# mqcomplab/bblean

Hardware: AMD Instinct MI355X
Metric: fingerprints/sec clustered (2048-bit, thr=0.3) (higher is better)
Workload: dtype u8

## Files before the change

bblean_amd/_engine.py:

```python
from __future__ import annotations

import ctypes as C
import os
import typing as tp

import numpy as np
from numpy.typing import NDArray

from bblean_amd import _lib

_WIDTH_DTYPES = {1: np.uint8, 2: np.uint16, 4: np.uint32, 8: np.uint64}


def _is_device_tensor(x: object) -> bool:
    return hasattr(x, "data_ptr") and getattr(x, "is_cuda", False)


def _launch_stream(x: object) -> int | None:
    if not _is_device_tensor(x):
        return None
    import torch

    return int(torch.cuda.current_stream(x.device).cuda_stream)

# ... 310 lines not shown
        out = np.empty((pos.size, self.nbytes), dtype=np.uint8)
        if pos.size:
            _lib.check(self._lib.bbh_tree_gather_centroids(self._h, pos.ctypes.data, pos.size, out.ctypes.data))
        return out

    def stats(self) -> NDArray[np.uint64]:
        out = np.zeros(8, dtype=np.uint64)
        _lib.check(self._lib.bbh_tree_stats(self._h, out.ctypes.data))
        return out

    def kernel_counts(self) -> NDArray[np.uint64]:
        out = np.zeros(8, dtype=np.uint64)
        _lib.check(self._lib.bbh_tree_kernel_counts(self._h, out.ctypes.data))
        return out

    def sys_counts(self) -> NDArray[np.uint64]:
        out = np.zeros(8, dtype=np.uint64)
        _lib.check(self._lib.bbh_tree_sys_counts(self._h, out.ctypes.data))
        return out

    def memory(self) -> NDArray[np.uint64]:
        out = np.zeros(8, dtype=np.uint64)
        _lib.check(self._lib.bbh_tree_memory(self._h, out.ctypes.data))
        return out

    def compact(self, seal: bool = True) -> None:
        _lib.check(self._lib.bbh_tree_compact(self._h, 1 if seal else 0))

    @staticmethod
    def image_min_stage(n_features: int) -> int:
# ... 49 lines not shown
```

bblean_amd/_lib.py:

```python
from __future__ import annotations

import ctypes as C
import os
from pathlib import Path

import numpy as np

_LIB: C.CDLL | None = None
_HERE = Path(__file__).resolve().parent

BBH_OK = 0
BBH_ERR_INVALID = 1
BBH_ERR_HIP = 2
BBH_ERR_NO_DEVICE = 3
BBH_ERR_CAPACITY = 4
BBH_ERR_STATE = 5
BBH_TOPK_MAX = 64

_vp = C.c_void_p
_i32 = C.c_int32
_i64 = C.c_int64
_f64 = C.c_double
_int = C.c_int

# ... 26 lines not shown
    ),
    "bbh_tree_create": (_int, [C.POINTER(_vp), _i32, _f64, _i32, _f64, _vp, _i64, _i32, _i32]),
    "bbh_tree_destroy": (_int, [_vp]),
    "bbh_tree_set_merge": (_int, [_vp, _i32, _f64, _vp, _i64, _f64, _i32]),
    "bbh_tree_reset": (_int, [_vp]),
    "bbh_tree_fit_packed": (_int, [_vp, _vp, _i64, _i64, _vp, _vp]),
    "bbh_tree_fit_buffers": (_int, [_vp, _vp, _i32, _i64, _vp, _vp]),
    "bbh_trees_fit_packed": (_int, [_vp, _i32, _vp, _vp, _vp, _vp, _vp]),
    "bbh_trees_fit_buffers": (_int, [_vp, _i32, _vp, _vp, _vp, _vp, _vp]),
    "bbh_tree_leaf_count": (_int, [_vp, C.POINTER(_i64)]),
    "bbh_tree_export_leaves": (_int, [_vp, _vp, _vp, _vp, _vp, _i32]),
    "bbh_tree_gather_buffers": (_int, [_vp, _vp, _i64, _i32, _vp]),
    "bbh_tree_gather_centroids": (_int, [_vp, _vp, _i64, _vp]),
    "bbh_tree_stats": (_int, [_vp, _vp]),
    "bbh_tree_kernel_counts": (_int, [_vp, _vp]),
    "bbh_tree_sys_counts": (_int, [_vp, _vp]),
    "bbh_tree_memory": (_int, [_vp, _vp]),
    "bbh_tree_compact": (_int, [_vp, _i32]),
    "bbh_tree_save_fd": (_int, [_vp, _int, C.c_uint64, C.POINTER(C.c_uint64)]),
    "bbh_tree_load_fd": (_int, [C.POINTER(_vp), _int, _i32, C.c_uint64]),
    "bbh_tree_image_check_fd": (_int, [_int, C.POINTER(C.c_uint64)]),
    "bbh_profile_enable": (_int, [_int]),
    "bbh_profile_reset": (_int, []),
    "bbh_profile_get": (_int, [C.c_char_p, C.POINTER(_i64), C.POINTER(_f64)]),
    "bbh_profile_units": (_int, [C.c_char_p, C.POINTER(_i64)]),
    "bbh_profile_longest": (_int, [C.c_char_p, C.POINTER(_f64), C.POINTER(_i64)]),
}

EXPORTED_SYMBOLS = tuple(_PROTOTYPES)

# ... 79 lines not shown
```

bblean_amd/csrc/bb_tree.hip:

```cpp
#include "bb_common.h"

#include <atomic>
#include <chrono>

#include <rocprim/device/device_scan.hpp>

#include <algorithm>
#include <cmath>
#include <future>
#include <type_traits>

using namespace bbd;

namespace {

constexpr int TB = 256;
constexpr int TW = TB / 64;
constexpr uint32_t NONE = 0xFFFFFFFFu;
constexpr int MAXD = 256;
constexpr int MAXFAST = 5;
constexpr int NRED = 2 + MAXFAST;
constexpr int MAX_BF = 1023;
constexpr int NPLW = 9;
constexpr int SPLIT_MLP = 16;
// ... 43 lines not shown
    uint32_t* node_link;
    RowMeta* node_rm;
    NodeHdr* node_hdr;
    uint8_t* scratch_cent;
    uint8_t* cf8;
    uint16_t* cf16;
    uint32_t* cf32;
    uint32_t cap_nodes, cap8, cap16, cap32;
    uint32_t ctr[C_COUNT];
    unsigned long long stats[8];
    unsigned long long phase[16];
    unsigned long long sphase[8];
    unsigned long long splitprof[10];
    unsigned long long mlprof[8];
    unsigned long long rprof[4];
    const uint8_t* rows;
    long long row_stride;
    const uint8_t* bufs;
    int32_t width;
    int32_t use_root_cache;
    long long n_elems;
    uint32_t* out_leaf;
    long long processed;
    int32_t stop_reason;
    int32_t audit;
    uint32_t giveup_line;
};

struct Smem {
    uint32_t x, vec, cA, cB;
// ... 2320 lines not shown
    if (!t->lazy_pools) {
        BB_HIP(hipMemset(h.node_hdr, 0, ((size_t)h.cap_nodes + 1) * sizeof(NodeHdr)));
        BB_TRY(write_empty_root(h));
    }
    h.ctr[C_NODES] = nblk;
    h.ctr[C_N8] = 1;
    h.ctr[C_ROOT] = 0;
    h.ctr[C_FIRST_LEAF] = 0;
    h.ctr[C_DEPTH] = 1;
    std::memset(h.stats, 0, sizeof(h.stats));
    std::memset(h.phase, 0, sizeof(h.phase));
    std::memset(h.sphase, 0, sizeof(h.sphase));
    std::memset(h.splitprof, 0, sizeof(h.splitprof));
    std::memset(h.mlprof, 0, sizeof(h.mlprof));
    std::memset(h.rprof, 0, sizeof(h.rprof));
    h.stats[5] = 1;
    t->chain_valid = false;
    t->pipe_ml = false;
    t->unsup_stretch = 0;
    return BBH_OK;
}

int set_tol(bbh_tree* t, const double* tab, int64_t len) {
    double* fresh = nullptr;
    if (tab && len > 0) {
        BB_HIP(bb::dev_alloc(&fresh, (size_t)len * 8));
        const hipError_t e = hipMemcpy(fresh, tab, (size_t)len * 8, hipMemcpyHostToDevice);
        if (e != hipSuccess) {
            (void)bb::dev_free(fresh);
            BB_HIP(e);
// ... 143 lines not shown
static void print_pipe_phases(const bbh_tree* t) {
    static const char* nm[16] = {"router:setup", "router:wait", "router:compare", "router:commit", "router:drain", "leaf:wait", "leaf:fill",
                                 "leaf:compare", "leaf:cf+dot", "leaf:decide+apply", "all:flush", "all:cold", "#runs", "#router-stale", "#leaf-pre-hits", "#leaf-stale"};
    const double n = (double)(t->h.stats[2] + t->h.stats[3]);
    fprintf(stderr, "[bbhip pipe phases, per insert]");
    for (int i = 0; i < 16; ++i) fprintf(stderr, " %s=%.*f", nm[i], i < 12 ? 0 : 4, n > 0 ? (double)t->h.phase[i] / n : 0.0);
    static const char* kd[3] = {"pre-compared, best row folded", "own", "pre-compared, every row checked"};
    fprintf(stderr, "\n[bbhip pipe leaf compares]");
    for (int i = 0; i < 3; ++i)
        fprintf(stderr, " %s: %.3f/insert x %.0f cycles", kd[i], n > 0 ? (double)t->h.sphase[2 * i + 1] / n : 0.0,
                t->h.sphase[2 * i + 1] ? (double)t->h.sphase[2 * i] / (double)t->h.sphase[2 * i + 1] : 0.0);
    fprintf(stderr, "\n");
    fprintf(stderr, "[bbhip pipe router waits, per insert] ring entry %.0f, row + pre-compare of wave 2 %.0f, pending jobs of a nearly full leaf %.0f, "
            "decision on a full leaf %.0f\n", n > 0 ? (double)t->h.rprof[0] / n : 0.0, n > 0 ? (double)t->h.rprof[1] / n : 0.0,
            n > 0 ? (double)t->h.rprof[2] / n : 0.0, n > 0 ? (double)t->h.rprof[3] / n : 0.0);
    if (t->h.splitprof[8]) {
        const double ns = (double)t->h.splitprof[8];
        fprintf(stderr, "[bbhip pipe leaf splits] %.4f/insert x %.0f cycles:", n > 0 ? ns / n : 0.0, (double)t->h.splitprof[9] / ns);
        for (int i = 0; i < 8; ++i) fprintf(stderr, " s%d=%.0f", i, (double)t->h.splitprof[i] / ns);
        fprintf(stderr, "\n");
    }
    if (t->pipe_ml)
        fprintf(stderr, "[bbhip pipe multi-level router] upper-slot fills %.3f/insert x %.0f cycles; tracking levels committed %.3f/insert, "
                "cluster-feature cache misses %.3f/insert; router waiting for a level's update by a helper wave %.0f cycles/insert, for "
                "all of them and their stores (before a fill) %.0f; of a fill: loads %.0f cycles, slot + corrections %.0f\n", n > 0 ? (double)t->h.sphase[7] / n : 0.0,
                t->h.sphase[7] ? (double)t->h.sphase[6] / (double)t->h.sphase[7] : 0.0, n > 0 ? (double)t->h.mlprof[1] / n : 0.0,
                n > 0 ? (double)t->h.mlprof[0] / n : 0.0, n > 0 ? (double)t->h.mlprof[2] / n : 0.0, n > 0 ? (double)t->h.mlprof[3] / n : 0.0,
                t->h.sphase[7] ? (double)t->h.mlprof[4] / (double)t->h.sphase[7] : 0.0, t->h.sphase[7] ? (double)t->h.mlprof[5] / (double)t->h.sphase[7] : 0.0);
}

// ... 232 lines not shown
            else if (left_midway == 0) multi_chunk = std::min<long long>(2 * multi_chunk, 1ll << 18);
        }

        for (size_t a = 0; a < active.size() && rc == BBH_OK; ++a) {
            Job& j = jobs[active[a]];
            bbh_tree* t = j.t;
            TreeDev& h = t->h;
            const TreeDev& back = harr[a];
            std::memcpy(h.ctr, back.ctr, sizeof(h.ctr));
            std::memcpy(h.stats, back.stats, sizeof(h.stats));
            std::memcpy(h.phase, back.phase, sizeof(h.phase));
            std::memcpy(h.sphase, back.sphase, sizeof(h.sphase));
            std::memcpy(h.splitprof, back.splitprof, sizeof(h.splitprof));
            std::memcpy(h.mlprof, back.mlprof, sizeof(h.mlprof));
            std::memcpy(h.rprof, back.rprof, sizeof(h.rprof));
            j.done += back.processed;
            t->kcount[label.kcol] += (uint64_t)back.processed;
            t->kcount[3 + label.kcol] += 1;
            if (engine == Engine::Sys) {
                rc = sys_after_launch(t, back, s);
                if (rc != BBH_OK) break;
            }
            const bool pool_stop = back.stop_reason == STOP_NODES || back.stop_reason == STOP_CF8 || back.stop_reason == STOP_CF16 || back.stop_reason == STOP_CF32;
            if (back.stop_reason == STOP_PIPE_UNSUPPORTED) t->kcount[6] += 1;
            if (pool_stop) t->kcount[7] += 1;
            if (j.old_left > 0) j.old_left = std::max<int64_t>(0, j.old_left - back.processed);
            if (t->sys_off_left > 0 && engine != Engine::Sys) t->sys_off_left = std::max<int64_t>(0, t->sys_off_left - back.processed);
            if (prof_tok != (size_t)-1) bb::prof_units(prof_tok, back.processed);
            j.stalls = (back.processed == 0 && back.stop_reason != STOP_PIPE_UNSUPPORTED && back.stop_reason != STOP_PIPE_NEEDS_ML) ? j.stalls + 1 : 0;
            if (j.stalls > 3) { rc = bb::fail(BBH_ERR_CAPACITY, "tree engine made no progress (stop reason %d)", back.stop_reason); break; }
// ... 497 lines not shown
}

extern "C" int bbh_tree_gather_centroids(bbh_tree* t, const int64_t* positions, int64_t m, uint8_t* out) {
    if (!t || (m > 0 && (!positions || !out))) return bb::fail(BBH_ERR_INVALID, "null argument");
    if (m < 0) return bb::fail(BBH_ERR_INVALID, "negative position count");
    if (m == 0) return BBH_OK;
    return gather_positions(t, positions, m, 0, nullptr, out);
}

extern "C" int bbh_tree_kernel_counts(bbh_tree* t, uint64_t* out8) {
    if (!t || !out8) return bb::fail(BBH_ERR_INVALID, "null argument");
    for (int i = 0; i < 8; ++i) out8[i] = t->kcount[i];
    return BBH_OK;
}

extern "C" int bbh_tree_sys_counts(bbh_tree* t, uint64_t* out8) {
    if (!t || !out8) return bb::fail(BBH_ERR_INVALID, "null argument");
    for (int i = 0; i < 8; ++i) out8[i] = t->syscount[i];
    return BBH_OK;
}

extern "C" int bbh_tree_memory(bbh_tree* t, uint64_t* out8) {
    if (!t || !out8) return bb::fail(BBH_ERR_INVALID, "null argument");
    const TreeDev& h = t->h;
    const size_t F = (size_t)h.F;
    out8[0] = (uint64_t)h.cap_nodes * block_bytes(h);
    out8[1] = (uint64_t)std::min(h.cap_nodes, h.ctr[C_NODES]) * block_bytes(h);
    out8[2] = (uint64_t)h.cap8 * F + (uint64_t)h.cap16 * F * 2 + (uint64_t)h.cap32 * F * 4;
    out8[3] = std::max(t->peak_bytes, pool_bytes(h));
    out8[4] = t->gc_runs;
// ... 31 lines not shown
```

bblean_amd/csrc/bb_tree_pipe.inc:

```

constexpr int PW_MAX = 8;
__host__ __device__ constexpr int pipe_pw(int bf) { return bf > 63 ? 4 : 8; }
__host__ __device__ constexpr int pipe_prew(int bf) { return bf > 63 ? 2 : 4; }
constexpr int PZ = 6;
constexpr int PNP = 12;
constexpr int PROMO_RESERVE = 1024;
constexpr int STOP_PIPE_UNSUPPORTED = 9;
constexpr int STOP_INTERNAL = 10;
constexpr int STOP_PIPE_NEEDS_ML = 11;
constexpr int STOP_PIPE_PREFERS_SL = 12;
#ifndef BBH_ML_STINT
#define BBH_ML_STINT 256
#endif
constexpr long long PIPE_ML_STINT = BBH_ML_STINT;
constexpr int PEMAX = 4;
constexpr uint32_t PRT = 16;

enum PipeReason : uint32_t { PR_DONE = 0, PR_COLD = 1, PR_STOP = 2, PR_UNSUP = 3, PR_FLUSH = 4, PR_ABORT = 5, PR_SPLIT = 6, PR_NEEDML = 7, PR_PREFSL = 8 };
enum PipeSplit : int { PS_LEAF = 0, PS_P, PS_JP, PS_LENP, PS_TRK, PS_POP, PS_XOFF, PS_SI };
enum PipeCtl : int { PC_HEAD = 0, PC_TAIL, PC_END, PC_ABORT, PC_REASON, PC_E_LO, PC_E_HI, PC_STOPCODE, PC_DCOUNT, PC_NZ, PC_PGO, PC_PLEN, PC_LGO, PC_PZERO,
                     PC_WM,
                     PC_COUNT };
static_assert(PC_COUNT <= 16, "the control block is 16 words");

struct PSmem {
    uint32_t x, ctr, stats;
    uint32_t ctl, ring, res, xq, delta, zrec;
    uint32_t mb, part;
    uint32_t srec;
    uint32_t llog, prec;
    uint32_t pver, lver, preP, preL, pst;
    int pw, prew;
    uint32_t leaf0, lslot_bytes, s_card, s_link, s_rm;
    uint32_t pslot, p_card, p_link, p_n, p_ts, p_clen, p_pend, pslot_bytes;
    uint32_t lrest;
    uint32_t cold_base, total;
    uint32_t cfc;
    uint32_t tcf;
    int nl, ncf, ntc;
    int nus;
    uint32_t upath, urt, urp;
};

__host__ __device__ constexpr PSmem pipe_layout(int bf, int ml = 0) {
    PSmem p{};
    const size_t rows = (size_t)bf + 1;
    p.x = 0; p.ctr = 256; p.stats = 256 + 64;
    uint32_t o = 256 + 64 + 64;
    p.ctl = o; o += 64;
    p.pw = pipe_pw(bf); p.prew = pipe_prew(bf);
    const uint32_t lanes4 = (uint32_t)((rows + 63) / 64 * 256);
    p.ring = o; o += p.pw * 16;
    p.res = o; o += p.pw * 4;
    p.xq = o; o += p.pw * 256;
    p.zrec = o; o += f_align16(PZ * 32);
    p.mb = o; o += 64;
    p.srec = o; o += 32;
    p.pst = o; o += 128;
    p.pver = o; o += lanes4;
    p.preP = o; o += p.prew * lanes4;
    p.part = o; o += 2 * (bf > 63 ? lanes4 : 0u);
    p.leaf0 = f_align16(o);
    p.s_card = f_align16(rows * FRBS);
    p.s_link = p.s_card + f_align16(rows * 4);
    p.s_rm = p.s_link + f_align16(rows * 4);
    p.lslot_bytes = p.s_rm + (uint32_t)(rows * 32);
    p.cold_base = p.leaf0 + p.lslot_bytes;
    p.pslot = p.cold_base;
    p.delta = p.pslot;
    p.p_card = f_align16(rows * FRBS);
    p.p_link = p.p_card + f_align16(rows * 4);
    p.p_n = p.p_link + f_align16(rows * 4);
    p.p_ts = p.p_n + f_align16(rows * 4);
    p.p_clen = p.p_ts + f_align16(rows * 4);
    p.p_pend = p.p_clen + f_align16(rows * 4);
    p.pslot_bytes = p.p_pend + f_align16(rows * 4);
    p.nus = ml ? PEMAX : 1;
    p.lrest = p.pslot + (uint32_t)p.nus * p.pslot_bytes;
    int nl = 1;
    while (nl < (ml ? 3 : 6) && (size_t)p.lrest + (size_t)nl * p.lslot_bytes <= 160 * 1024) ++nl;
    p.nl = nl;
    const uint32_t cold = smem_layout(bf, 256, 0).total;
    const uint32_t end_slots = p.lrest + (uint32_t)(nl - 1) * p.lslot_bytes;
    p.lver = f_align16(end_slots);
    p.preL = bf > 63 ? p.preP : p.lver + (uint32_t)nl * lanes4;
    p.cfc = p.lver + (uint32_t)nl * lanes4 + (bf > 63 ? 0u : (uint32_t)p.prew * lanes4);
    const uint32_t lim = 160 * 1024 - (bf > 63 ? 64u * 7u : 0u) - (ml ? (uint32_t)(PEMAX * 32 + PRT * 8 + PW_MAX * 4 + 64) : 0u);
    int ncf = p.cfc < lim ? (int)((lim - p.cfc) / 2048) : 0;
    p.ncf = ncf > 8 ? 8 : ncf;
    p.tcf = p.cfc + (uint32_t)p.ncf * 2048;
    int ntc = p.tcf < lim ? (int)((lim - p.tcf) / 8192) : 0;
    p.ntc = ntc > 4 ? 4 : (ntc < 0 ? 0 : ntc);
    p.llog = p.tcf + (uint32_t)p.ntc * 8192;
    p.prec = p.llog + 64 * (uint32_t)nl;
    uint32_t end_all = p.prec + 64;
    if (ml) {
        p.upath = end_all;
        p.urt = p.upath + PEMAX * 32;
        p.urp = p.urt + PRT * 8;
        end_all = p.urp + PW_MAX * 4;
    }
    const uint32_t end_cold = p.cold_base + cold;
    p.total = end_all > end_cold ? end_all : end_cold;
    return p;
}

__host__ __device__ constexpr FSmem pipe_fsmem(int bf) {
    const PSmem p = pipe_layout(bf);
    FSmem f{};
    f.x = p.x; f.ctr = p.ctr; f.stats = p.stats;
    f.slot0 = p.leaf0; f.slot_bytes = p.lslot_bytes; f.s_card = p.s_card; f.s_link = p.s_link; f.s_rm = p.s_rm;
    f.cold_base = p.cold_base; f.total = p.total; f.ns = p.nl; f.npp = 0; f.cold_slot = 1;
    return f;
}

static_assert(pipe_layout(50).total <= 160 * 1024, "bf 50 must fit");
static_assert(pipe_layout(254).total <= 160 * 1024, "bf 254 must fit");
static_assert(pipe_layout(50, 1).total <= 160 * 1024 && pipe_layout(50, 1).ntc >= 3 && pipe_layout(50, 1).ncf >= 4 && pipe_layout(50, 1).nl >= 3,
              "bf 50, several exact levels: four upper slots, three leaf slots and the caches must fit");
static_assert(pipe_layout(50, 1).leaf0 == pipe_layout(50).leaf0 && pipe_layout(50, 1).cold_base == pipe_layout(50).cold_base &&
              pipe_layout(50, 1).lslot_bytes == pipe_layout(50).lslot_bytes, "one cold layout per branching factor");

#if defined(__HIPCC__)

#define PIPE_SPIN_LIMIT (1u << 22)
#define PIPE_MARK() ((void)0)
__device__ unsigned int g_pipe_audit = 0;
__device__ unsigned long long g_pipe_audit_runs = 0;
#define PIPE_AUDIT_FAIL(code) atomicCAS(&g_pipe_audit, 0u, ((unsigned)(code) << 16) | (unsigned)__LINE__)
#define PIPE_CBAR() asm volatile("" ::: "memory")

template <int BF>
struct KColdP : KCBase {
    static constexpr bool dynamic_shape = false;
    static constexpr int F = 2048, nb = 256, RB = 256, RBc = 16, RBS = (int)FRBS;
    static constexpr uint32_t rows = BF + 1, bf = BF, nblk = node_blocks(BF + 1);
    static constexpr int nm = 1;
    static constexpr Smem o = smem_layout_cold(BF, pipe_fsmem(BF));
};

template <int BF>
__device__ __attribute__((noinline)) void cold_insert_one_p(unsigned char* smem_raw, TreeDev* T, long long e) {
    tree_insert_body<false, KColdP<BF>, true>(smem_raw, T, e);
}

template <int BF, bool PROF = false>
__device__ __attribute__((noinline)) void cold_leaf_split_p(unsigned char* smem_raw, TreeDev* T, long long e, uint32_t pcx, uint32_t leafnode,
                                                            uint32_t P, uint32_t jp, uint32_t lenP, uint32_t trk) {
    const u64 sp_t0 = PROF ? __builtin_amdgcn_s_memtime() : 0;
    constexpr FSmem f = pipe_fsmem(BF);
    KColdS<BF> k;
    k.cent = T->node_cent; k.card = T->node_card; k.link = T->node_link; k.rm = T->node_rm; k.hdr = T->node_hdr;
    k.scratch = T->scratch_cent; k.cf8 = T->cf8; k.cf16 = T->cf16; k.cf32 = T->cf32;
    k.bufs = nullptr; k.width = 0;
    k.crit = 0; k.tol_len = 0; k.thr = 0; k.tolerance = 0; k.tol = nullptr;
    k.L = (LA unsigned char*)smem_raw;
    k.o = smem_layout_cold(BF, f);
    const int tid = threadIdx.x;
    LA uint32_t* lctr = (LA uint32_t*)(k.L + f.ctr);
    LA uint32_t* bc = lds<uint32_t>(k.L, k.o.bc);
    Elem el;
    el.idx = e; el.nS = 1; el.s1S = 0; el.s2S = 0; el.pcx = pcx;
    __syncthreads();
    uint32_t cN = uni(lctr[C_NODES]), c32 = uni(lctr[C_N32]), cFirst = uni(lctr[C_FIRST_LEAF]);
    int red_slot = 0, cmp_par = 0;
    u64 sph[8] = {0, 0, 0, 0, 0, 0, 0, 0};
    split_node<false, PROF>(k, el, red_slot, cmp_par, leafnode, 0u, true, trk, cN, c32, cFirst, T->ctr, sph);
    const uint32_t node1 = uni(bc[0]), cardA = uni(bc[3]), cardB = uni(bc[4]);
    const uint32_t nA = uni(bc[7]), nB = uni(bc[8]);
    const uint32_t slotA = (2u << 30) | uni(bc[9]), slotB = (2u << 30) | uni(bc[10]);
    const uint32_t bad = uni(bc[11]);
    node_put_row(k, P, jp, k.o.cA, cardA, node1, NONE, nA, slotA, 0, 0);
    node_put_row(k, P, lenP, k.o.cB, cardB, leafnode, NONE, nB, slotB, 0, 0);
    if (tid == 0) {
        stg<uint32_t>(k.hdr + P, lenP + 1);
        lctr[C_NODES] = cN; lctr[C_N32] = c32; lctr[C_FIRST_LEAF] = cFirst;
        lctr[8] = bad ? (uint32_t)STOP_RANGE : (uint32_t)STOP_DONE;
    }
    __syncthreads();
    if constexpr (PROF) {
        if (tid == 0) {
            for (int i = 0; i < 8; ++i) T->splitprof[i] += sph[i];
            T->splitprof[8] += 1;
            T->splitprof[9] += __builtin_amdgcn_s_memtime() - sp_t0;
        }
    }
}

// ... 740 lines not shown
    for (int i = 0; i < 32; ++i) { tx[i] = 0; ty[i] = 0; }
    uint32_t xtag = NONE, xts = 0, ytag = NONE, yts = 0;
    bool curx = false;
    constexpr int NTC = p.ntc;
    uint32_t ttag[NTC > 0 ? NTC : 1], tts[NTC > 0 ? NTC : 1], tuse[NTC > 0 ? NTC : 1];
#pragma unroll
    for (int c = 0; c < (NTC > 0 ? NTC : 1); ++c) { ttag[c] = NONE; tts[c] = 0; tuse[c] = 0; }

    uint32_t Z = 0, zrows = 0, P = NONE, plen = 0;
    constexpr bool RV = RPL == 1;
    uint32_t r_link = NONE, r_n = 0, r_ts = 0, r_clen = 0, r_pend = 0, r_card = 0, r_ver = 0;
    (void)r_link; (void)r_n; (void)r_ts; (void)r_clen; (void)r_pend; (void)r_card; (void)r_ver;
    uint32_t budget = (1u << PNP) - 1;
    bool ok = depth >= 2 && depth - 2 <= (uint32_t)PZ;
    bool needml = false;
    {
        uint32_t nd = cRoot;
#pragma unroll 1
        for (uint32_t z = 0; ok && z + 2 < depth; ++z) {
            const size_t m = (size_t)nd * NG;
            const uint32_t len = uni(ldg<uint32_t>(g_hdr + nd));
            bool any = false;
#pragma unroll
            for (int q = 0; q < RPL; ++q) {
                const uint32_t r = (uint32_t)q * 64 + lane;
                const uint32_t rc = r < rows ? r : rows - 1;
                const uint32_t cd = ldg<uint32_t>(g_card + m + rc);
                any = any || (r < len && cd != 0);
            }
            const u32x4_t r0 = ldg<u32x4_t>((const uint8_t*)(g_rm + m));
            const uint32_t l0 = uni(ldg<uint32_t>(g_link + m));
// ... 9 lines not shown
            const uint32_t zn = uni(zr[0]), zn_at = uni(zr[2]), zfd = uni(zr[3]);
            if (zn == nd && uni(zr[1]) == ts0 && n0 >= zn_at && zfd > (n0 - zn_at) + 64u) {
                fd = zfd - (n0 - zn_at);
            } else {
                uint32_t v[32];
                cf32_lane_load(g_cf32, ts0, lane, v);
                uint32_t mn = 0xFFFFFFFFu;
#pragma unroll
                for (int i = 0; i < 32; ++i) {
                    const uint32_t d = 2u * v[i] < n0 ? n0 - 2u * v[i] : 0u;
                    mn = d < mn ? d : mn;
                }
                fd = wmin32(mn);
                if (lane == 0) { zr[2] = n0; zr[3] = fd; }
            }
            if (lane == 0) { zr[0] = nd; zr[1] = ts0; }
            const uint32_t room = fd > 0 ? fd - 1 : 0;
            budget = room < budget ? room : budget;
            zrows += len;
            nd = l0;
            Z = z + 1;
        }
        P = nd;
    }
    if (!ok) {
        reason = needml ? PR_NEEDML : PR_UNSUP;
    } else if (budget == 0) {
        reason = PR_COLD;
    } else {
        const size_t pm = (size_t)P * NG;
        const u32x2_t hraw = ldg<u32x2_t>(g_hdr + P);
        pipe_fill_rows<K, 0, PFill<K>::NIT>(L, p.pslot, g_cent, P);
        uint32_t lk[RPL];
#pragma unroll
        for (int q = 0; q < RPL; ++q) {
            const uint32_t r = (uint32_t)q * 64 + lane;
            const uint32_t rc = r < rows ? r : rows - 1;
            const uint32_t cd = ldg<uint32_t>(g_card + pm + rc);
            lk[q] = ldg<uint32_t>(g_link + pm + rc);
            const u32x2_t ns = ldg<u32x2_t>((const uint8_t*)(g_rm + pm + rc) + 4);
// ... 29 lines not shown
                const uint32_t rc = r < rows ? r : rows - 1;
                uint32_t cl = bf + 1, clf = 1;
                if (r < plen) {
                    const u32x2_t ch = ldg<u32x2_t>(g_hdr + lk[q]);
                    cl = hw_cap(ch.y) < rows ? bf + 1 : ch.x; clf = ch.y & HW_LEAF;
                }
                bad = bad || clf == 0;
                *(LA uint32_t*)(L + p.pslot + p.p_clen + rc * 4) = cl;
                if constexpr (RV) r_clen = cl;
            }
            if (__ballot(bad) != 0ull) reason = PR_UNSUP;
        }
    }

    pph<PROF>(pr, 0);
    if constexpr (PROF) pr.ph[12] += 1;
    const bool pzero = nzc == 0;
    if (reason == PR_DONE) {
#pragma unroll
        for (int q = 0; q < RPL; ++q) *(LA uint32_t*)(L + p.pver + ((uint32_t)q * 64 + lane) * 4) = 0u;
        if (lane < 8) *(LA uint32_t*)(L + p.pst + lane * 4) = 0u;
        if (lane == 0) {
            *(LA uint32_t*)(L + p.ctl + PC_PLEN * 4) = plen;
            *(LA uint32_t*)(L + p.ctl + PC_PZERO * 4) = pzero ? 1u : 0u;
        }
        PIPE_CBAR();
        lds_st(L, p.ctl + PC_PGO * 4, 1u);
        uint32_t tail_seen = 0;
        auto retire_to_tail = [&]() {
            const uint32_t t = tail_seen;
            PIPE_CBAR();
// ... 258 lines not shown
            if (T->audit != 0 && reason != PR_ABORT) {
                retire_poll();
                asm volatile("s_waitcnt vmcnt(0)" ::: "memory");
                if constexpr (RV) {
                    if (lane < rows) {
                        *(LA uint32_t*)(L + p.pslot + p.p_card + lane * 4) = r_card;
                        *(LA uint32_t*)(L + p.pslot + p.p_n + lane * 4) = r_n;
                        *(LA uint32_t*)(L + p.pslot + p.p_link + lane * 4) = r_link;
                        *(LA uint32_t*)(L + p.pslot + p.p_clen + lane * 4) = r_clen;
                        *(LA uint32_t*)(L + p.pslot + p.p_pend + lane * 4) = r_pend;
                    }
                }
                PIPE_CBAR();
                if (T->audit == 2 && lane == 0) *(LA uint32_t*)(L + p.pslot) ^= 1u;
                pipe_audit_tracking_slot<K>(L, T, p.pslot, P, plen, reason != PR_SPLIT);
            }
        }
        if (xtag != NONE) cf32_lane_store(g_cf32, xts, lane, tx);
        if (ytag != NONE) cf32_lane_store(g_cf32, yts, lane, ty);
#pragma unroll
        for (int c = 0; c < NTC; ++c) {
            if (ttag[c] != NONE) {
                uint32_t* dst = g_cf32 + (size_t)(tts[c] & 0x3FFFFFFFu) * 2048 + (size_t)lane * 32;
#pragma unroll
                for (int g = 0; g < 8; ++g) stg<u32x4_t>(dst + g * 4, *(LA u32x4_t*)(L + p.tcf + (uint32_t)c * 8192 + ((uint32_t)g * 64 + lane) * 16));
            }
        }
#pragma unroll
        for (int k = 0; k < PNP; ++k) *(LA uint32_t*)(L + p.delta + k * 256 + lane * 4) = dp[k];
        pph<PROF>(pr, 4);
// ... 79 lines not shown
        for (uint32_t w = 0; w < 2; ++w) {
            uint32_t spins = 0;
            while (uni(lds_ld(L, p.mb + (CQ_FIN + w) * 4)) != cposted) {
                if (uni(lds_ld(L, p.ctl + PC_ABORT * 4)) != 0u || ++spins > PIPE_SPIN_LIMIT) { lost_c = true; PIPE_MARK(); break; }
            }
        }
        PIPE_CBAR();
        cseen = 0xFFu;
        if constexpr (PROF) cwa_cycles += __builtin_amdgcn_s_memtime() - t0_;
    };
    uint32_t utag = NONE, ulen = 0, uuse = 0, uclock = 0;

    uint32_t Z = 0, zrows = 0, top = NONE;
    uint32_t budget = (1u << PNP) - 1;
    bool ok = depth >= 2;
    {
        uint32_t nd = cRoot;
#pragma unroll 1
        for (uint32_t z = 0; ok && z + 2 < depth && z < (uint32_t)PZ; ++z) {
            const size_t m = (size_t)nd * NG;
            const uint32_t len = uni(ldg<uint32_t>(g_hdr + nd));
            const uint32_t rc = lane < rows ? lane : rows - 1;
            const uint32_t cd = ldg<uint32_t>(g_card + m + rc);
            const bool any = lane < len && cd != 0;
            const u32x4_t r0 = ldg<u32x4_t>((const uint8_t*)(g_rm + m));
            const uint32_t l0 = uni(ldg<uint32_t>(g_link + m));
            if (len == 0) { ok = false; break; }
            if (__ballot(any) != 0ull) break;
            const uint32_t n0 = uni(r0.y), ts0 = uni(r0.z);
            if (n0 >= 0x7FFF0000u) { ok = false; break; }
// ... 2 lines not shown
            const uint32_t zn = uni(zr[0]), zn_at = uni(zr[2]), zfd = uni(zr[3]);
            if (zn == nd && uni(zr[1]) == ts0 && n0 >= zn_at && zfd > (n0 - zn_at) + 64u) {
                fd = zfd - (n0 - zn_at);
            } else {
                uint32_t v[32];
                cf32_lane_load(g_cf32, ts0, lane, v);
                uint32_t mn = 0xFFFFFFFFu;
#pragma unroll
                for (int i = 0; i < 32; ++i) {
                    const uint32_t d = 2u * v[i] < n0 ? n0 - 2u * v[i] : 0u;
                    mn = d < mn ? d : mn;
                }
                fd = wmin32(mn);
                if (lane == 0) { zr[2] = n0; zr[3] = fd; }
            }
            if (lane == 0) { zr[0] = nd; zr[1] = ts0; }
            const uint32_t room = fd > 0 ? fd - 1 : 0;
            budget = room < budget ? room : budget;
            zrows += len;
            nd = l0;
            Z = z + 1;
        }
        top = nd;
    }
    const uint32_t E = ok ? depth - 1 - Z : 0u;

    u64 fprof[2] = {0, 0};
    (void)fprof;
    bool fill_sealed = false;
    auto fill_slot = [&](uint32_t si, uint32_t nd, bool plevel, bool midrun, uint32_t l) -> bool {
        const uint32_t sb = p.pslot + si * p.pslot_bytes;
// ... 894 lines not shown
__device__ __forceinline__ void pipe_flush_delta(LA unsigned char* L, TreeDev* T) {
    constexpr PSmem p = K::p;
    const int tid = threadIdx.x;
    LA uint32_t* ctl = (LA uint32_t*)(L + p.ctl);
    const uint32_t cnt = uni(ctl[PC_DCOUNT]), nz = uni(ctl[PC_NZ]);
    if (cnt == 0 || nz == 0) return;
    uint32_t v[8] = {0, 0, 0, 0, 0, 0, 0, 0};
#pragma unroll
    for (int k = 0; k < PNP; ++k) {
        const uint32_t byte = *(LA uint8_t*)(L + p.delta + k * 256 + tid);
#pragma unroll
        for (int q = 0; q < 8; ++q) v[q] |= ((byte >> (7 - q)) & 1u) << k;
    }
    uint32_t* const g_cf32 = T->cf32;
    RowMeta* const g_rm = T->node_rm;
#pragma unroll 1
    for (uint32_t z = 0; z < nz; ++z) {
        LA uint32_t* zr = (LA uint32_t*)(L + p.zrec + z * 32);
        const uint32_t nd = uni(zr[0]), ts = uni(zr[1]);
        uint32_t* cf = g_cf32 + (size_t)(ts & 0x3FFFFFFFu) * 2048 + (size_t)tid * 8;
        u32x4_t q0 = ldg<u32x4_t>(cf), q1 = ldg<u32x4_t>(cf + 4);
        q0.x += v[0]; q0.y += v[1]; q0.z += v[2]; q0.w += v[3];
        q1.x += v[4]; q1.y += v[5]; q1.z += v[6]; q1.w += v[7];
        stg<u32x4_t>(cf, q0);
        stg<u32x4_t>(cf + 4, q1);
        if (tid == 0) {
            uint8_t* rm = (uint8_t*)(g_rm + (size_t)nd * NG);
            const uint32_t n0 = ldg<uint32_t>(rm + 4);
            stg<uint32_t>(rm + 4, n0 + cnt);
            stg<uint32_t>(rm + 12, 0u);
        }
    }
}

template <class K, bool PROF>
__device__ __forceinline__ void tree_pipe_body(unsigned char* smem_raw, TreeDev* T) {
    constexpr PSmem p = K::p;
    LA unsigned char* L = (LA unsigned char*)smem_raw;
    const int tid = threadIdx.x;
    const uint32_t wave = uni((uint32_t)tid >> 6);
    LA uint32_t* lctr = (LA uint32_t*)(L + p.ctr);
    LA u64* lstats = (LA u64*)(L + p.stats);
    LA uint32_t* ctl = (LA uint32_t*)(L + p.ctl);
    if (tid < C_COUNT) lctr[tid] = T->ctr[tid];
    if (tid == 8) lctr[8] = STOP_DONE;
    if (tid < 8) lstats[tid] = T->stats[tid];
    if (tid < 16) ((LA u32x4_t*)(L + p.x))[tid] = (u32x4_t)(0);
    if (tid < PZ * 8) ((LA uint32_t*)(L + p.zrec))[tid] = NONE;
    __syncthreads();
    const long long n_elems = T->n_elems;
    long long e = 0;
    int stop = STOP_DONE;
    while (e < n_elems) {
        if (tid < 16) ctl[tid] = 0u;
        if (tid >= 16 && tid < 32) ((LA uint32_t*)(L + p.mb))[tid - 16] = 0u;
        __syncthreads();
        if (wave == 0) {
            if constexpr (K::ML) pipe_router_ml<K, PROF>(L, T, e);
            else pipe_router<K, PROF>(L, T, e);
        }
        else if (wave == 1) {
            if constexpr (K::RPL == 1) {
                pipe_leaf<K, PROF, false>(L, T);
// ... 37 lines not shown
        if constexpr (PROF) { if (tid == 0) T->phase[10] += c1 - c0; }
        if (reason == PR_DONE) break;
        if (reason == PR_FLUSH) continue;
        if (reason == PR_SPLIT) {
            LA uint32_t* sp = (LA uint32_t*)(L + p.srec);
            const uint32_t s_leaf = uni(sp[PS_LEAF]), s_P = uni(sp[PS_P]), s_jp = uni(sp[PS_JP]), s_lenP = uni(sp[PS_LENP]);
            const uint32_t s_trk = uni(sp[PS_TRK]), s_pop = uni(sp[PS_POP]), s_xoff = uni(sp[PS_XOFF]), s_si = uni(sp[PS_SI]);
            __syncthreads();
            if (s_si != 0) {
                const uint32_t src = p.lrest + (s_si - 1) * p.lslot_bytes;
                for (uint32_t i = (uint32_t)tid; i < p.lslot_bytes / 16; i += TB)
                    *(LA u32x4_t*)(L + p.leaf0 + i * 16) = *(LA u32x4_t*)(L + src + i * 16);
            }
            if (tid < 64) ((LA uint32_t*)(L + p.x))[tid] = *(LA uint32_t*)(L + s_xoff + tid * 4);
            __syncthreads();
            cold_leaf_split_p<K::BF, PROF>(smem_raw, T, e - 1, s_pop, s_leaf, s_P, s_jp, s_lenP, s_trk);
            if constexpr (PROF) { if (tid == 0) { T->phase[11] += __builtin_amdgcn_s_memtime() - c1; } }
            const uint32_t sstop = uni(lctr[8]);
            __syncthreads();
            if (sstop != STOP_DONE) { stop = (int)sstop; break; }
            continue;
        }
        if (reason == PR_STOP) { stop = (int)uni(ctl[PC_STOPCODE]); break; }
        if (reason == PR_UNSUP) { stop = STOP_PIPE_UNSUPPORTED; break; }
        if (reason == PR_NEEDML) { stop = STOP_PIPE_NEEDS_ML; break; }
        if (reason == PR_PREFSL) { stop = STOP_PIPE_PREFERS_SL; break; }
        if (reason == PR_ABORT) {
            if (tid == 0) T->giveup_line = uni(ctl[PC_ABORT]);
            stop = STOP_INTERNAL;
            break;
        }
        if (e >= n_elems) break;
        cold_insert_one_p<K::BF>(smem_raw, T, e);
        const uint32_t cstop = uni(lctr[8]), cdone = uni(lctr[9]);
        if (tid < PZ * 8) ((LA uint32_t*)(L + p.zrec))[tid] = NONE;
        __syncthreads();
        if constexpr (PROF) { if (tid == 0) T->phase[11] += __builtin_amdgcn_s_memtime() - c1; }
        if (cstop != STOP_DONE || cdone == 0) { stop = (int)cstop; break; }
        e += 1;
    }
    __syncthreads();
    if (tid < C_COUNT) T->ctr[tid] = lctr[tid];
    if (tid < 8) T->stats[tid] = lstats[tid];
    if (tid == 0) {
        T->processed = e;
        T->stop_reason = stop;
    }
}

template <class K, bool PROF = false>
__global__ __launch_bounds__(TB) __attribute__((amdgpu_waves_per_eu(1, 1))) void k_tree_pipe(TreeDev* trees) {
    extern __shared__ __align__(16) unsigned char smem_raw[];
    tree_pipe_body<K, PROF>(smem_raw, trees + blockIdx.x);
}

#endif
```

include/bbhip.h:

```cpp
#ifndef BBHIP_H
#define BBHIP_H

#include <stddef.h>
#include <stdint.h>

#ifdef __cplusplus
extern "C" {
#endif

#define BBH_OK 0
#define BBH_ERR_INVALID 1
#define BBH_ERR_HIP 2
#define BBH_ERR_NO_DEVICE 3
#define BBH_ERR_CAPACITY 4
#define BBH_ERR_STATE 5

#define BBH_CRIT_DIAMETER 0
#define BBH_CRIT_RADIUS 1
#define BBH_CRIT_TOL_DIAMETER 2
#define BBH_CRIT_TOL_RADIUS 3
#define BBH_CRIT_TOL_LEGACY 4
#define BBH_CRIT_NEVER 5

const char* bbh_last_error(void);
// ... 94 lines not shown

int bbh_tree_leaf_count(bbh_tree* t, int64_t* out);

int bbh_tree_export_leaves(bbh_tree* t, uint32_t* leaf_ids, uint64_t* n_samples,
                           uint8_t* packed_centroids, void* linear_sums, int32_t ls_width);

int bbh_tree_gather_buffers(bbh_tree* t, const int64_t* positions, int64_t m,
                            int32_t width, void* out);

int bbh_tree_gather_centroids(bbh_tree* t, const int64_t* positions, int64_t m, uint8_t* out);

int bbh_tree_stats(bbh_tree* t, uint64_t* out8);

int bbh_tree_kernel_counts(bbh_tree* t, uint64_t* out8);

int bbh_tree_sys_counts(bbh_tree* t, uint64_t* out8);

int bbh_tree_memory(bbh_tree* t, uint64_t* out8);

int bbh_tree_compact(bbh_tree* t, int32_t seal);

#define BBH_TREE_IMAGE_MIN_STAGE(n_features) \
    ((uint64_t)64 * (4 * ((((uint64_t)(n_features) / 8) + 15) / 16 * 16) + 176))
int bbh_tree_save_fd(bbh_tree* t, int fd, uint64_t stage_bytes, uint64_t* written);
int bbh_tree_load_fd(bbh_tree** out, int fd, int32_t device, uint64_t stage_bytes);
int bbh_tree_image_check_fd(int fd, uint64_t* image_bytes);

int bbh_profile_enable(int on);
int bbh_profile_reset(void);
int bbh_profile_get(const char* name, int64_t* launches, double* total_ms);
// ... 8 lines not shown
```

Before: 460,600.

## Keep leaf-parent slot warm in LDS across leaf splits and flushes

After a leaf split or flush, the pipe kernel now saves the leaf-parent's row data and path records in a reserved LDS area, so the next run can start from LDS instead of walking the tree again from HBM. The LDS layout is rearranged so the cold scratch either sits after the parent slot or overlays only its tail rows, which are refetched when needed. The split routine writes its updated rows straight into the warm slot. The per-level counter update is also restructured to issue all cf32 loads before the adds and to reuse cached counts instead of reloading them, and counters for warm and cold run starts are added. The risks are extra LDS pressure and harder-to-check validity of the cached state.

```diff
diff --git a/bblean_amd/_engine.py b/bblean_amd/_engine.py
--- a/bblean_amd/_engine.py
+++ b/bblean_amd/_engine.py
@@ -348,6 +348,11 @@
         _lib.check(self._lib.bbh_tree_kernel_counts(self._h, out.ctypes.data))
         return out
 
+    def pipe_run_starts(self) -> NDArray[np.uint64]:
+        out = np.zeros(2, dtype=np.uint64)
+        _lib.check(self._lib.bbh_tree_pipe_run_starts(self._h, out.ctypes.data))
+        return out
+
     def sys_counts(self) -> NDArray[np.uint64]:
         out = np.zeros(8, dtype=np.uint64)
         _lib.check(self._lib.bbh_tree_sys_counts(self._h, out.ctypes.data))
diff --git a/bblean_amd/_lib.py b/bblean_amd/_lib.py
--- a/bblean_amd/_lib.py
+++ b/bblean_amd/_lib.py
@@ -64,6 +64,7 @@
     "bbh_tree_gather_centroids": (_int, [_vp, _vp, _i64, _vp]),
     "bbh_tree_stats": (_int, [_vp, _vp]),
     "bbh_tree_kernel_counts": (_int, [_vp, _vp]),
+    "bbh_tree_pipe_run_starts": (_int, [_vp, _vp]),
     "bbh_tree_sys_counts": (_int, [_vp, _vp]),
     "bbh_tree_memory": (_int, [_vp, _vp]),
     "bbh_tree_compact": (_int, [_vp, _i32]),
diff --git a/bblean_amd/csrc/bb_tree.hip b/bblean_amd/csrc/bb_tree.hip
--- a/bblean_amd/csrc/bb_tree.hip
+++ b/bblean_amd/csrc/bb_tree.hip
@@ -81,6 +81,7 @@
     unsigned long long splitprof[10];
     unsigned long long mlprof[8];
     unsigned long long rprof[4];
+    unsigned long long runstarts[4];
     const uint8_t* rows;
     long long row_stride;
     const uint8_t* bufs;
@@ -2431,6 +2432,7 @@
     std::memset(h.splitprof, 0, sizeof(h.splitprof));
     std::memset(h.mlprof, 0, sizeof(h.mlprof));
     std::memset(h.rprof, 0, sizeof(h.rprof));
+    std::memset(h.runstarts, 0, sizeof(h.runstarts));
     h.stats[5] = 1;
     t->chain_valid = false;
     t->pipe_ml = false;
@@ -2604,6 +2606,9 @@
     fprintf(stderr, "[bbhip pipe router waits, per insert] ring entry %.0f, row + pre-compare of wave 2 %.0f, pending jobs of a nearly full leaf %.0f, "
             "decision on a full leaf %.0f\n", n > 0 ? (double)t->h.rprof[0] / n : 0.0, n > 0 ? (double)t->h.rprof[1] / n : 0.0,
             n > 0 ? (double)t->h.rprof[2] / n : 0.0, n > 0 ? (double)t->h.rprof[3] / n : 0.0);
+    fprintf(stderr, "[bbhip pipe run starts] warm (from LDS, after a leaf split or a flush) %llu x %.0f cycles, cold (from HBM) %llu x %.0f cycles\n",
+            (unsigned long long)t->h.runstarts[0], t->h.runstarts[0] ? (double)t->h.runstarts[2] / (double)t->h.runstarts[0] : 0.0,
+            (unsigned long long)t->h.runstarts[1], t->h.runstarts[1] ? (double)t->h.runstarts[3] / (double)t->h.runstarts[1] : 0.0);
     if (t->h.splitprof[8]) {
         const double ns = (double)t->h.splitprof[8];
         fprintf(stderr, "[bbhip pipe leaf splits] %.4f/insert x %.0f cycles:", n > 0 ? ns / n : 0.0, (double)t->h.splitprof[9] / ns);
@@ -2866,6 +2871,7 @@
             std::memcpy(h.splitprof, back.splitprof, sizeof(h.splitprof));
             std::memcpy(h.mlprof, back.mlprof, sizeof(h.mlprof));
             std::memcpy(h.rprof, back.rprof, sizeof(h.rprof));
+            std::memcpy(h.runstarts, back.runstarts, sizeof(h.runstarts));
             j.done += back.processed;
             t->kcount[label.kcol] += (uint64_t)back.processed;
             t->kcount[3 + label.kcol] += 1;
@@ -3393,6 +3399,13 @@
     return BBH_OK;
 }
 
+extern "C" int bbh_tree_pipe_run_starts(bbh_tree* t, uint64_t* out2) {
+    if (!t || !out2) return bb::fail(BBH_ERR_INVALID, "null argument");
+    out2[0] = t->h.runstarts[0];
+    out2[1] = t->h.runstarts[1];
+    return BBH_OK;
+}
+
 extern "C" int bbh_tree_sys_counts(bbh_tree* t, uint64_t* out8) {
     if (!t || !out8) return bb::fail(BBH_ERR_INVALID, "null argument");
     for (int i = 0; i < 8; ++i) out8[i] = t->syscount[i];
diff --git a/bblean_amd/csrc/bb_tree_pipe.inc b/bblean_amd/csrc/bb_tree_pipe.inc
--- a/bblean_amd/csrc/bb_tree_pipe.inc
+++ b/bblean_amd/csrc/bb_tree_pipe.inc
@@ -18,6 +18,7 @@
 
 enum PipeReason : uint32_t { PR_DONE = 0, PR_COLD = 1, PR_STOP = 2, PR_UNSUP = 3, PR_FLUSH = 4, PR_ABORT = 5, PR_SPLIT = 6, PR_NEEDML = 7, PR_PREFSL = 8 };
 enum PipeSplit : int { PS_LEAF = 0, PS_P, PS_JP, PS_LENP, PS_TRK, PS_POP, PS_XOFF, PS_SI };
+enum PipeWarm : int { PWR_P = 0, PWR_Z, PWR_ZROWS, PWR_PLEN, PWR_ROOT, PWR_NWARM, PWR_NCOLD };
 enum PipeCtl : int { PC_HEAD = 0, PC_TAIL, PC_END, PC_ABORT, PC_REASON, PC_E_LO, PC_E_HI, PC_STOPCODE, PC_DCOUNT, PC_NZ, PC_PGO, PC_PLEN, PC_LGO, PC_PZERO,
                      PC_WM,
                      PC_COUNT };
@@ -28,6 +29,7 @@
     uint32_t ctl, ring, res, xq, delta, zrec;
     uint32_t mb, part;
     uint32_t srec;
+    uint32_t wrec;
     uint32_t llog, prec;
     uint32_t pver, lver, preP, preL, pst;
     int pw, prew;
@@ -35,6 +37,8 @@
     uint32_t pslot, p_card, p_link, p_n, p_ts, p_clen, p_pend, pslot_bytes;
     uint32_t lrest;
     uint32_t cold_base, total;
+    int warm;
+    uint32_t wrow0;
     uint32_t cfc;
     uint32_t tcf;
     int nl, ncf, ntc;
@@ -56,6 +60,7 @@
     p.zrec = o; o += f_align16(PZ * 32);
     p.mb = o; o += 64;
     p.srec = o; o += 32;
+    p.wrec = o; o += 32;
     p.pst = o; o += 128;
     p.pver = o; o += lanes4;
     p.preP = o; o += p.prew * lanes4;
@@ -65,9 +70,7 @@
     p.s_link = p.s_card + f_align16(rows * 4);
     p.s_rm = p.s_link + f_align16(rows * 4);
     p.lslot_bytes = p.s_rm + (uint32_t)(rows * 32);
-    p.cold_base = p.leaf0 + p.lslot_bytes;
-    p.pslot = p.cold_base;
-    p.delta = p.pslot;
+    p.pslot = p.leaf0 + p.lslot_bytes;
     p.p_card = f_align16(rows * FRBS);
     p.p_link = p.p_card + f_align16(rows * 4);
     p.p_n = p.p_link + f_align16(rows * 4);
@@ -75,12 +78,16 @@
     p.p_clen = p.p_ts + f_align16(rows * 4);
     p.p_pend = p.p_clen + f_align16(rows * 4);
     p.pslot_bytes = p.p_pend + f_align16(rows * 4);
+    const uint32_t cold = smem_layout(bf, 256, 0).total;
+    p.warm = (size_t)p.pslot + p.pslot_bytes + cold <= 160 * 1024 ? 1 : (!ml && rows * FRBS >= cold ? 2 : 0);
+    p.cold_base = p.warm == 1 ? p.pslot + p.pslot_bytes : p.warm == 2 ? p.pslot + (uint32_t)((rows * FRBS - cold) / 16 * 16) : p.pslot;
+    p.wrow0 = p.warm == 2 ? (p.cold_base - p.pslot) / FRBS : (uint32_t)rows;
+    p.delta = ml ? p.pslot : p.cold_base;
     p.nus = ml ? PEMAX : 1;
     p.lrest = p.pslot + (uint32_t)p.nus * p.pslot_bytes;
     int nl = 1;
     while (nl < (ml ? 3 : 6) && (size_t)p.lrest + (size_t)nl * p.lslot_bytes <= 160 * 1024) ++nl;
     p.nl = nl;
-    const uint32_t cold = smem_layout(bf, 256, 0).total;
     const uint32_t end_slots = p.lrest + (uint32_t)(nl - 1) * p.lslot_bytes;
     p.lver = f_align16(end_slots);
     p.preL = bf > 63 ? p.preP : p.lver + (uint32_t)nl * lanes4;
@@ -99,6 +106,9 @@
         p.urt = p.upath + PEMAX * 32;
         p.urp = p.urt + PRT * 8;
         end_all = p.urp + PW_MAX * 4;
+    } else if (p.warm == 1) {
+        p.delta = end_all;
+        end_all += PNP * 256;
     }
     const uint32_t end_cold = p.cold_base + cold;
     p.total = end_all > end_cold ? end_all : end_cold;
@@ -116,6 +126,10 @@
 
 static_assert(pipe_layout(50).total <= 160 * 1024, "bf 50 must fit");
 static_assert(pipe_layout(254).total <= 160 * 1024, "bf 254 must fit");
+static_assert(pipe_layout(254).warm == 2 && pipe_layout(254).wrow0 >= 64 && pipe_layout(254).nl == 1 &&
+              pipe_layout(254).cold_base + smem_layout(254, 256, 0).total <= pipe_layout(254).pslot + pipe_layout(254).p_card,
+              "bf 254: the scratch overlays the end of the leaf-parent's row area only");
+static_assert(pipe_layout(50).warm == 1 && pipe_layout(50).nl == 6 && pipe_layout(50).ntc == 3, "bf 50: the leaf-parent's slot survives a leaf split at no cost in slots or caches");
 static_assert(pipe_layout(50, 1).total <= 160 * 1024 && pipe_layout(50, 1).ntc >= 3 && pipe_layout(50, 1).ncf >= 4 && pipe_layout(50, 1).nl >= 3,
               "bf 50, several exact levels: four upper slots, three leaf slots and the caches must fit");
 static_assert(pipe_layout(50, 1).leaf0 == pipe_layout(50).leaf0 && pipe_layout(50, 1).cold_base == pipe_layout(50).cold_base &&
@@ -144,7 +158,7 @@
     tree_insert_body<false, KColdP<BF>, true>(smem_raw, T, e);
 }
 
-template <int BF, bool PROF = false>
+template <int BF, bool PROF = false, bool WARM = false>
 __device__ __attribute__((noinline)) void cold_leaf_split_p(unsigned char* smem_raw, TreeDev* T, long long e, uint32_t pcx, uint32_t leafnode,
                                                             uint32_t P, uint32_t jp, uint32_t lenP, uint32_t trk) {
     const u64 sp_t0 = PROF ? __builtin_amdgcn_s_memtime() : 0;
@@ -172,6 +186,31 @@
     const uint32_t bad = uni(bc[11]);
     node_put_row(k, P, jp, k.o.cA, cardA, node1, NONE, nA, slotA, 0, 0);
     node_put_row(k, P, lenP, k.o.cB, cardB, leafnode, NONE, nB, slotB, 0, 0);
+    if constexpr (WARM) {
+        constexpr PSmem p = pipe_layout(BF);
+        static_assert(p.warm != 0 && p.cold_base >= p.pslot + p.wrow0 * FRBS, "the scratch must not overlay the slot's first wrow0 rows");
+        if (tid < 128) {
+            const uint32_t row = tid < 64 ? jp : lenP, src = tid < 64 ? k.o.cA : k.o.cB;
+            if (row < p.wrow0)
+                *(LA uint32_t*)(k.L + p.pslot + row * FRBS + ((uint32_t)tid & 63u) * 4) = *(LA uint32_t*)(k.L + src + ((uint32_t)tid & 63u) * 4);
+        }
+        if (tid == 0) {
+            const uint32_t n1 = bc[5], n2 = bc[6];
+            auto put = [&](uint32_t row, uint32_t card, uint32_t link, uint32_t n, uint32_t slot, uint32_t clen) {
+                *(LA uint32_t*)(k.L + p.pslot + p.p_card + row * 4) = card;
+                *(LA uint32_t*)(k.L + p.pslot + p.p_link + row * 4) = link;
+                *(LA uint32_t*)(k.L + p.pslot + p.p_n + row * 4) = n;
+                *(LA uint32_t*)(k.L + p.pslot + p.p_ts + row * 4) = slot;
+                *(LA uint32_t*)(k.L + p.pslot + p.p_clen + row * 4) = clen;
+                *(LA uint32_t*)(k.L + p.pslot + p.p_pend + row * 4) = 0u;
+            };
+            put(jp, cardA, node1, nA, slotA, n1);
+            put(lenP, cardB, leafnode, nB, slotB, n2);
+            LA uint32_t* wr = (LA uint32_t*)(k.L + p.wrec);
+            wr[PWR_PLEN] = lenP + 1;
+            if (bad) wr[PWR_P] = NONE;
+        }
+    }
     if (tid == 0) {
         stg<uint32_t>(k.hdr + P, lenP + 1);
         lctr[C_NODES] = cN; lctr[C_N32] = c32; lctr[C_FIRST_LEAF] = cFirst;
@@ -942,7 +981,57 @@
     uint32_t budget = (1u << PNP) - 1;
     bool ok = depth >= 2 && depth - 2 <= (uint32_t)PZ;
     bool needml = false;
-    {
+    bool warm = false;
+    if constexpr (p.warm != 0) {
+        LA uint32_t* wr = (LA uint32_t*)(L + p.wrec);
+        const u32x4_t w4 = lds_ld4(L, p.wrec);
+        const uint32_t wP = uni(w4.x), wZ = uni(w4.y), wzrows = uni(w4.z), wplen = uni(w4.w), wroot = uni(wr[PWR_ROOT]);
+        PIPE_CBAR();
+        if (lane == 0) wr[PWR_P] = NONE;
+        if (ok && wP != NONE && wZ + 2 == depth && wroot == cRoot) {
+            uint32_t b = budget;
+            bool good = true;
+#pragma unroll 1
+            for (uint32_t z = 0; z < wZ; ++z) {
+                const u32x4_t zc = lds_ld4(L, p.zrec + z * 32);
+                const uint32_t zn_at = uni(zc.z), zfd = uni(zc.w), n0 = uni(lds_ld(L, p.zrec + z * 32 + 16));
+                if (uni(zc.x) == NONE || n0 >= 0x7FFF0000u || n0 < zn_at || zfd <= (n0 - zn_at) + 64u) { good = false; break; }
+                const uint32_t fd = zfd - (n0 - zn_at);
+                const uint32_t room = fd > 0 ? fd - 1 : 0;
+                b = room < b ? room : b;
+            }
+            if (good && b != 0) {
+                warm = true;
+                budget = b; Z = wZ; zrows = wzrows; P = wP; plen = wplen;
+                if constexpr (RV) {
+                    const uint32_t rc = lane < rows ? lane : rows - 1;
+                    r_card = *(LA uint32_t*)(L + p.pslot + p.p_card + rc * 4);
+                    r_link = *(LA uint32_t*)(L + p.pslot + p.p_link + rc * 4);
+                    r_n = *(LA uint32_t*)(L + p.pslot + p.p_n + rc * 4);
+                    r_ts = *(LA uint32_t*)(L + p.pslot + p.p_ts + rc * 4);
+                    r_clen = *(LA uint32_t*)(L + p.pslot + p.p_clen + rc * 4);
+                    r_pend = 0u; r_ver = 0u;
+                    nzc = wsum32((lane < plen && r_card != 0u) ? 1u : 0u);
+                } else {
+                    if constexpr (p.warm == 2) {
+                        constexpr int I0 = (int)(p.wrow0 * 16 / 64);
+                        static_assert(I0 < PFill<K>::NIT, "the scratch overlays some rows");
+                        if (plen > p.wrow0) pipe_fill_rows<K, I0, PFill<K>::NIT>(L, p.pslot, g_cent, P);
+                    }
+                    uint32_t nzl = 0;
+#pragma unroll
+                    for (int q = 0; q < RPL; ++q) {
+                        const uint32_t r = (uint32_t)q * 64 + lane;
+                        const uint32_t rc = r < rows ? r : rows - 1;
+                        nzl += (r < plen && *(LA uint32_t*)(L + p.pslot + p.p_card + rc * 4) != 0u) ? 1u : 0u;
+                    }
+                    nzc = wsum32(nzl);
+                }
+            }
+        }
+    }
+    if (lane == 0) ((LA uint32_t*)(L + p.wrec))[warm ? PWR_NWARM : PWR_NCOLD] += 1u;
+    if (!warm) {
         uint32_t nd = cRoot;
 #pragma unroll 1
         for (uint32_t z = 0; ok && z + 2 < depth; ++z) {
@@ -982,7 +1071,7 @@
                 fd = wmin32(mn);
                 if (lane == 0) { zr[2] = n0; zr[3] = fd; }
             }
-            if (lane == 0) { zr[0] = nd; zr[1] = ts0; }
+            if (lane == 0) { zr[0] = nd; zr[1] = ts0; zr[4] = n0; }
             const uint32_t room = fd > 0 ? fd - 1 : 0;
             budget = room < budget ? room : budget;
             zrows += len;
@@ -991,7 +1080,8 @@
         }
         P = nd;
     }
-    if (!ok) {
+    if (warm) {
+    } else if (!ok) {
         reason = needml ? PR_NEEDML : PR_UNSUP;
     } else if (budget == 0) {
         reason = PR_COLD;
@@ -1051,7 +1141,10 @@
     }
 
     pph<PROF>(pr, 0);
-    if constexpr (PROF) pr.ph[12] += 1;
+    if constexpr (PROF) {
+        pr.ph[12] += 1;
+        if (lane == 0) atomicAdd((unsigned long long*)&T->runstarts[warm ? 2 : 3], (unsigned long long)pr.ph[0]);
+    }
     const bool pzero = nzc == 0;
     if (reason == PR_DONE) {
 #pragma unroll
@@ -1340,6 +1433,25 @@
                 PIPE_CBAR();
                 if (T->audit == 2 && lane == 0) *(LA uint32_t*)(L + p.pslot) ^= 1u;
                 pipe_audit_tracking_slot<K>(L, T, p.pslot, P, plen, reason != PR_SPLIT);
+            }
+        }
+        if constexpr (p.warm != 0) {
+            if (reason == PR_SPLIT || reason == PR_FLUSH) {
+                retire_poll();
+                if constexpr (RV) {
+                    if (lane < rows) {
+                        *(LA uint32_t*)(L + p.pslot + p.p_card + lane * 4) = r_card;
+                        *(LA uint32_t*)(L + p.pslot + p.p_n + lane * 4) = r_n;
+                        *(LA uint32_t*)(L + p.pslot + p.p_link + lane * 4) = r_link;
+                        *(LA uint32_t*)(L + p.pslot + p.p_ts + lane * 4) = r_ts;
+                        *(LA uint32_t*)(L + p.pslot + p.p_clen + lane * 4) = r_clen;
+                    }
+                }
+                if (lane == 0) {
+                    LA uint32_t* wr = (LA uint32_t*)(L + p.wrec);
+                    wr[PWR_Z] = Z; wr[PWR_ZROWS] = zrows; wr[PWR_PLEN] = plen; wr[PWR_ROOT] = cRoot;
+                    wr[PWR_P] = P;
+                }
             }
         }
         if (xtag != NONE) cf32_lane_store(g_cf32, xts, lane, tx);
@@ -1449,6 +1561,7 @@
     uint32_t Z = 0, zrows = 0, top = NONE;
     uint32_t budget = (1u << PNP) - 1;
     bool ok = depth >= 2;
+    if (lane == 0) ((LA uint32_t*)(L + p.wrec))[PWR_NCOLD] += 1u;
     {
         uint32_t nd = cRoot;
 #pragma unroll 1
@@ -1481,7 +1594,7 @@
                 fd = wmin32(mn);
                 if (lane == 0) { zr[2] = n0; zr[3] = fd; }
             }
-            if (lane == 0) { zr[0] = nd; zr[1] = ts0; }
+            if (lane == 0) { zr[0] = nd; zr[1] = ts0; zr[4] = n0; }
             const uint32_t room = fd > 0 ? fd - 1 : 0;
             budget = room < budget ? room : budget;
             zrows += len;
@@ -2406,20 +2519,33 @@
     }
     uint32_t* const g_cf32 = T->cf32;
     RowMeta* const g_rm = T->node_rm;
+    uint32_t* cf[PZ];
+    u32x4_t q0[PZ], q1[PZ];
+#pragma unroll
+    for (uint32_t z = 0; z < (uint32_t)PZ; ++z) {
+        const uint32_t zc = z < nz ? z : nz - 1;
+        const uint32_t ts = uni(*(LA uint32_t*)(L + p.zrec + zc * 32 + 4));
+        cf[z] = g_cf32 + (size_t)(ts & 0x3FFFFFFFu) * 2048 + (size_t)tid * 8;
+        if (z < nz) { q0[z] = ldg<u32x4_t>(cf[z]); q1[z] = ldg<u32x4_t>(cf[z] + 4); }
+    }
+#pragma unroll
+    for (uint32_t z = 0; z < (uint32_t)PZ; ++z) {
+        if (z < nz) {
+            u32x4_t a = q0[z], b = q1[z];
+            a.x += v[0]; a.y += v[1]; a.z += v[2]; a.w += v[3];
+            b.x += v[4]; b.y += v[5]; b.z += v[6]; b.w += v[7];
+            stg<u32x4_t>(cf[z], a);
+            stg<u32x4_t>(cf[z] + 4, b);
+        }
+    }
+    if (tid == 0) {
 #pragma unroll 1
-    for (uint32_t z = 0; z < nz; ++z) {
-        LA uint32_t* zr = (LA uint32_t*)(L + p.zrec + z * 32);
-        const uint32_t nd = uni(zr[0]), ts = uni(zr[1]);
-        uint32_t* cf = g_cf32 + (size_t)(ts & 0x3FFFFFFFu) * 2048 + (size_t)tid * 8;
-        u32x4_t q0 = ldg<u32x4_t>(cf), q1 = ldg<u32x4_t>(cf + 4);
-        q0.x += v[0]; q0.y += v[1]; q0.z += v[2]; q0.w += v[3];
-        q1.x += v[4]; q1.y += v[5]; q1.z += v[6]; q1.w += v[7];
-        stg<u32x4_t>(cf, q0);
-        stg<u32x4_t>(cf + 4, q1);
-        if (tid == 0) {
-            uint8_t* rm = (uint8_t*)(g_rm + (size_t)nd * NG);
-            const uint32_t n0 = ldg<uint32_t>(rm + 4);
-            stg<uint32_t>(rm + 4, n0 + cnt);
+        for (uint32_t z = 0; z < nz; ++z) {
+            LA uint32_t* zr = (LA uint32_t*)(L + p.zrec + z * 32);
+            uint8_t* rm = (uint8_t*)(g_rm + (size_t)zr[0] * NG);
+            const uint32_t n1 = zr[4] + cnt;
+            zr[4] = n1;
+            stg<uint32_t>(rm + 4, n1);
             stg<uint32_t>(rm + 12, 0u);
         }
     }
@@ -2439,6 +2565,7 @@
     if (tid < 8) lstats[tid] = T->stats[tid];
     if (tid < 16) ((LA u32x4_t*)(L + p.x))[tid] = (u32x4_t)(0);
     if (tid < PZ * 8) ((LA uint32_t*)(L + p.zrec))[tid] = NONE;
+    if (tid >= 64 && tid < 72) ((LA uint32_t*)(L + p.wrec))[tid - 64] = tid == 64 + PWR_P ? NONE : 0u;
     __syncthreads();
     const long long n_elems = T->n_elems;
     long long e = 0;
@@ -2506,7 +2633,7 @@
             }
             if (tid < 64) ((LA uint32_t*)(L + p.x))[tid] = *(LA uint32_t*)(L + s_xoff + tid * 4);
             __syncthreads();
-            cold_leaf_split_p<K::BF, PROF>(smem_raw, T, e - 1, s_pop, s_leaf, s_P, s_jp, s_lenP, s_trk);
+            cold_leaf_split_p<K::BF, PROF, !K::ML && p.warm != 0>(smem_raw, T, e - 1, s_pop, s_leaf, s_P, s_jp, s_lenP, s_trk);
             if constexpr (PROF) { if (tid == 0) { T->phase[11] += __builtin_amdgcn_s_memtime() - c1; } }
             const uint32_t sstop = uni(lctr[8]);
             __syncthreads();
@@ -2537,6 +2664,8 @@
     if (tid == 0) {
         T->processed = e;
         T->stop_reason = stop;
+        T->runstarts[0] += ((LA uint32_t*)(L + p.wrec))[PWR_NWARM];
+        T->runstarts[1] += ((LA uint32_t*)(L + p.wrec))[PWR_NCOLD];
     }
 }
 
diff --git a/include/bbhip.h b/include/bbhip.h
--- a/include/bbhip.h
+++ b/include/bbhip.h
@@ -132,6 +132,8 @@
 
 int bbh_tree_kernel_counts(bbh_tree* t, uint64_t* out8);
 
+int bbh_tree_pipe_run_starts(bbh_tree* t, uint64_t* out2);
+
 int bbh_tree_sys_counts(bbh_tree* t, uint64_t* out8);
 
 int bbh_tree_memory(bbh_tree* t, uint64_t* out8);
```

After: 462,400, median of 6. No clear change (+0.4%).
